# cychomatica/AudioPure

Measured on AMD Instinct MI355X. Metric: purified 1s@16kHz utterances/sec at 5 reverse steps, higher is better.
Workload: dtype f32

## Files before the change

audiopure_amd/csrc/ap_resblock_f32w.hip:

```cpp
#include "ap_common.h"

#include <type_traits>

namespace ap {

namespace {

constexpr int WC_ = 256;
constexpr int NP_ = 32;
constexpr int KCW_ = 32;
constexpr int NCH_ = WC_ / KCW_;
constexpr int XS_ = KCW_ + 4;
constexpr int XCOMP_ = NP_ * XS_;
constexpr int XBUF_ = 4 * XCOMP_;
constexpr int GS_ = WC_ + 4;
constexpr int GOFF_ = 2 * XBUF_;
constexpr int POFF_ = GOFF_ + 64 * GS_;
constexpr int PS_ = 36;
constexpr int LDS_FLOATS_ = GOFF_ + 64 * GS_;
constexpr int LDS_FLOATS_Q16_ = POFF_ + 4 * 2 * 32 * PS_;
constexpr int NCONST_ = 5 * WC_;
constexpr int DIET_CARRY_ = 2;
constexpr int DIET_CONST_ = 4;
constexpr int DIET_ROWS_ = 16;
constexpr int DIET_PK_ = 32;
constexpr int DIET_ZERO_ = 128;
constexpr int DIET_SEAM_ = 1024;
#ifndef AP_F32W_DIET
#define AP_F32W_DIET 1206
#endif
constexpr int DIET4_ = 0;
constexpr unsigned UNIT_BYTES_ = 4 * 64 * 16;
constexpr unsigned W1W_WAVE_BYTES_ = NCH_ * 4 * 4 * UNIT_BYTES_;
constexpr unsigned W2W_WAVE_BYTES_ = (WC_ / 8) * UNIT_BYTES_;

}

__global__ void pack_w1w_kernel(const float *__restrict__ w1f, float *__restrict__ out) {
  constexpr int C = WC_;
  const unsigned idx = blockIdx.x * blockDim.x + threadIdx.x;
  if (idx >= 4u * NCH_ * 4 * 4 * 4 * 64 * 4) return;
  const int e = idx & 3, lane = (idx >> 2) & 63, rt = (idx >> 8) & 3, comp = (idx >> 10) & 3, kg = (idx >> 12) & 3,
            ch = (idx >> 14) & 7, w = idx >> 17;
  const int i = lane & 31, hh = lane >> 5;
  const int c = 32 * ch + 8 * kg + 4 * hh + e;
  const int o = (rt & 1) * C + 64 * w + 32 * (rt >> 1) + i;
  const float *p = w1f + ((size_t)o * C + c) * 3;
  const double w0 = p[0], w1 = p[1], w2 = p[2];
  const double v = comp == 0 ? w0 : comp == 1 ? (w0 + w1 + w2) * 0.5 : comp == 2 ? (w0 - w1 + w2) * 0.5 : w2;
  out[idx] = (float)v;
}

__global__ void pack_w2w_kernel(const float *__restrict__ w2f, float *__restrict__ out) {
  constexpr int C = WC_;
  const unsigned idx = blockIdx.x * blockDim.x + threadIdx.x;
  if (idx >= 4u * (C / 8) * 4 * 64 * 4) return;
  const int e = idx & 3, lane = (idx >> 2) & 63, rt = (idx >> 8) & 3, kg = (idx >> 10) & 31, w = idx >> 15;
  const int i = lane & 31, hh = lane >> 5;
  const int c = 8 * kg + 4 * hh + e;
  const int o = (rt >> 1) * C + 64 * w + 32 * (rt & 1) + i;
  out[idx] = w2f[(size_t)o * C + c];
}

int launch_pack_f32w(ap_ctx *ctx, hipStream_t st) {
  const int C = ctx->C, S = ctx->S;
  const size_t n1f = (size_t)2 * C * C * 3, n2 = (size_t)(C + S) * C, n1w = (size_t)4 * 2 * C * C;
  for (int n = 0; n < ctx->NL; n++) {
    pack_w1w_kernel<<<(unsigned)((n1w + 255) / 256), 256, 0, st>>>(ctx->w1f + n * n1f, ctx->w1w + n * n1w);
    pack_w2w_kernel<<<(unsigned)((n2 + 255) / 256), 256, 0, st>>>(ctx->w2f + n * n2, ctx->w2w + n * n2);
  }
  AP_HIP(hipGetLastError());
  return 0;
}

template <bool NOH, bool SAVE = false, bool Q16 = false, int DIET = AP_F32W_DIET>
__global__ __launch_bounds__(256, 1) void resblock_f32w_kernel(
    const float *__restrict__ hin, const float *__restrict__ pt, float *__restrict__ hout, float *__restrict__ skip,
    const float *__restrict__ w1w, const float *__restrict__ b1, const float *__restrict__ w2w,
    const float *__restrict__ b2, int L, int logd, int accumulate, int ntiles, int nblk, float *__restrict__ aout) {
  constexpr int C = WC_;
  constexpr bool CARRY = (DIET & DIET_CARRY_) != 0, CONST = (DIET & DIET_CONST_) != 0;
  constexpr bool ROWS = Q16 && !NOH && (DIET & DIET_ROWS_) != 0;
  constexpr bool PK = Q16 && (DIET & DIET_PK_) != 0;
  constexpr bool ZERO = Q16 && (DIET & DIET_ZERO_) != 0;
  constexpr bool SEAM = Q16 && (DIET & DIET_SEAM_) != 0;
  static_assert(!SEAM || (CARRY && ZERO), "DIET_SEAM_ is written for the peeled first and last chunk");
  constexpr int COFF_ = Q16 ? LDS_FLOATS_Q16_ : LDS_FLOATS_;
  __shared__ __attribute__((aligned(16))) float lds[COFF_ + (CONST ? NCONST_ : 0)];

  const int tid = threadIdx.x;
  const int lane = tid & 63;
  const int wave = __builtin_amdgcn_readfirstlane(tid >> 6);
  const int j = lane & 31, hh = lane >> 5;
  const int sq = tid >> 5;
  const int d = 1 << logd;

  int t_first, t_step, t_end;
  {
    const int g = blockIdx.x, G = gridDim.x;
    if (G >= 8 && (G & 7) == 0) {
      const int xcd = g & 7, idx = g >> 3, q = nblk >> 3, r = nblk & 7;
      const int base = xcd < r ? xcd * (q + 1) : r * (q + 1) + (xcd - r) * q;
      t_first = base + idx;
      t_step = G >> 3;
      t_end = base + q + (xcd < r ? 1 : 0);
    } else {
      t_first = g;
      t_step = G;
      t_end = nblk;
    }
  }
  if (t_first >= t_end) return;
  if constexpr (CONST) {
    for (int i = tid; i < NCONST_; i += 256) lds[COFF_ + i] = i < 2 * C ? b1[i] : i < 4 * C ? b2[i - 2 * C] : pt[i - 4 * C];
    __syncthreads();
  }

  auto uni_rsrc = [&](const void *base, unsigned bytes) {
    const uint64_t hb = (uint64_t)base;
    const uint32_t lo = __builtin_amdgcn_readfirstlane((uint32_t)hb);
    const uint32_t hi = __builtin_amdgcn_readfirstlane((uint32_t)(hb >> 32));
    return __builtin_amdgcn_make_buffer_rsrc((void *)(((uint64_t)hi << 32) | lo), 0, (int)bytes, 0x00020000);
  };
  const unsigned clip_bytes = (unsigned)C * (unsigned)L * 4u;
  const __amdgpu_buffer_rsrc_t w1rs = uni_rsrc(reinterpret_cast<const char *>(w1w) + (size_t)wave * W1W_WAVE_BYTES_, W1W_WAVE_BYTES_);
  const __amdgpu_buffer_rsrc_t w2rs = uni_rsrc(reinterpret_cast<const char *>(w2w) + (size_t)wave * W2W_WAVE_BYTES_, W2W_WAVE_BYTES_);
  const unsigned lane16 = (unsigned)lane * 16u;
  const __amdgpu_buffer_rsrc_t b1rs = uni_rsrc(b1, 2u * C * 4u), b2rs = uni_rsrc(b2, 2u * C * 4u), ptrs = uni_rsrc(pt, C * 4u);
  auto ld4 = [&](const __amdgpu_buffer_rsrc_t &rs, int idx) {
    return __builtin_bit_cast(f32x4, __builtin_amdgcn_raw_buffer_load_b128(rs, (unsigned)idx * 4u, 0, 0));
  };
  int cbase = COFF_ + 64 * wave + 4 * hh;
  if constexpr (CONST && ROWS) asm volatile("" : "+v"(cbase));
  auto ld_c = [&](int idx) {
    if constexpr (ROWS) return *reinterpret_cast<const f32x4 *>(lds + cbase + (idx - 64 * wave - 4 * hh));
    else return *reinterpret_cast<const f32x4 *>(lds + COFF_ + idx);
  };
  auto ld_b1 = [&](int idx) { if constexpr (CONST) return ld_c(idx); else return ld4(b1rs, idx); };
  auto ld_b2 = [&](int idx) { if constexpr (CONST) return ld_c(2 * C + idx); else return ld4(b2rs, idx); };
  auto ld_pt = [&](int idx) { if constexpr (CONST) return ld_c(4 * C + idx); else return ld4(ptrs, idx); };

  auto load_a1 = [&](f32x4(&a)[4], unsigned unit) {
#pragma unroll
    for (int rt = 0; rt < 4; rt++)
      a[rt] = __builtin_bit_cast(f32x4, __builtin_amdgcn_raw_buffer_load_b128(w1rs, lane16 + rt * 1024u, unit * UNIT_BYTES_, 0));
  };
  auto load_a2 = [&](f32x4(&a)[4], unsigned kg) {
#pragma unroll
    for (int rt = 0; rt < 4; rt++)
      a[rt] = __builtin_bit_cast(f32x4, __builtin_amdgcn_raw_buffer_load_b128(w2rs, lane16 + rt * 1024u, kg * UNIT_BYTES_, 0));
  };

  const int col0 = d >= 32 ? j : (((j >> logd) << (logd + 1)) + (j & (d - 1)));
  const int col1 = d >= 32 ? 32 + j : col0 + d;

  int b, p0;
  __amdgpu_buffer_rsrc_t hrs;
  unsigned voff[4];
  bool tok[4];
  auto set_tile = [&](int tile) {
    b = __builtin_amdgcn_readfirstlane(tile / ntiles);
    p0 = __builtin_amdgcn_readfirstlane((tile % ntiles) * NP_);
    hrs = uni_rsrc(hin + (size_t)b * C * L, clip_bytes);
    const int p = p0 + j;
    const int tf = ((p >> logd) << (logd + 1)) + (p & (d - 1));
#pragma unroll
    for (int k = 0; k < 4; k++) {
      const int tp = tf + (k - 1) * d;
      tok[k] = (tp >= 0) && (tp < L);
      voff[k] = ((unsigned)min(max(tp, 0), L - 1) + (unsigned)(4 * sq) * (unsigned)L) * 4u;
    }
  };
    float xr[4][4];
    f32x4 ptq;
    auto issue_x = [&](int ch) {
      ptq = __builtin_bit_cast(f32x4, __builtin_amdgcn_raw_buffer_load_b128(ptrs, (unsigned)(16 * sq), ch * KCW_ * 4, 0));
#pragma unroll
      for (int cc = 0; cc < 4; cc++)
#pragma unroll
        for (int k = 0; k < 4; k++)
          xr[cc][k] = __builtin_bit_cast(float, __builtin_amdgcn_raw_buffer_load_b32(hrs, voff[k], (ch * KCW_ + cc) * L * 4, 0));
    };
    auto store_x = [&](float *dst) {
      asm volatile("" : "+v"(xr[0][0]), "+v"(xr[0][1]), "+v"(xr[0][2]), "+v"(xr[0][3]), "+v"(xr[1][0]), "+v"(xr[1][1]), "+v"(xr[1][2]),
                   "+v"(xr[1][3]), "+v"(xr[2][0]), "+v"(xr[2][1]), "+v"(xr[2][2]), "+v"(xr[2][3]), "+v"(xr[3][0]), "+v"(xr[3][1]),
                   "+v"(xr[3][2]), "+v"(xr[3][3]), "+v"(ptq));
      f32x4 c0, c1, c2, c3;
#pragma unroll
      for (int cc = 0; cc < 4; cc++) {
        const float u0 = tok[0] ? xr[cc][0] + ptq[cc] : 0.f;
        const float u1 = tok[1] ? xr[cc][1] + ptq[cc] : 0.f;
        const float u2 = tok[2] ? xr[cc][2] + ptq[cc] : 0.f;
        const float u3 = tok[3] ? xr[cc][3] + ptq[cc] : 0.f;
        c0[cc] = u0 - u2;
        c1[cc] = u1 + u2;
        c2[cc] = u2 - u1;
        c3[cc] = u3 - u1;
      }
      float *q = dst + j * XS_ + 4 * sq;
      *reinterpret_cast<f32x4 *>(q) = c0;
      *reinterpret_cast<f32x4 *>(q + XCOMP_) = c1;
      *reinterpret_cast<f32x4 *>(q + 2 * XCOMP_) = c2;
      *reinterpret_cast<f32x4 *>(q + 3 * XCOMP_) = c3;
    };

    f32x4 a[4][4];
    set_tile(t_first);
#pragma unroll
    for (int u = 0; u < 4; u++) load_a1(a[u], (unsigned)u);
    issue_x(0);

#pragma unroll 1
  for (int tile = t_first; tile < t_end; tile += t_step) {
    f32x16 acc[4][4];
    const float *xfrag = lds + j * XS_ + 4 * hh;
    f32x4 bqc[2];
    if constexpr (SEAM) {
      store_x(lds);
      __syncthreads();
      bqc[0] = *reinterpret_cast<const f32x4 *>(xfrag);
      __builtin_amdgcn_sched_barrier(0);
    }
#pragma unroll
    for (int rt = 0; rt < 4; rt++) {
      const int obase = (rt & 1) * C + 64 * wave + 32 * (rt >> 1);
#pragma unroll
      for (int q = 0; q < 4; q++) {
        const f32x4 bv = ld_b1(obase + 8 * q + 4 * hh);
        acc[1][rt][4 * q + 0] = bv[0];
        acc[1][rt][4 * q + 1] = bv[1];
        acc[1][rt][4 * q + 2] = bv[2];
        acc[1][rt][4 * q + 3] = bv[3];
      }
      if constexpr (!ZERO) {
#pragma unroll
        for (int r = 0; r < 16; r++) acc[0][rt][r] = acc[2][rt][r] = acc[3][rt][r] = 0.f;
      }
    }
    if constexpr (!SEAM) {
      store_x(lds);
      __syncthreads();
    }

    constexpr int NSTAGE = CARRY ? NCH_ - 1 : NCH_;
    auto chunk = [&](int ch, auto stage_tag, auto first_tag) __attribute__((always_inline)) {
      constexpr bool STAGE = decltype(stage_tag)::value, FIRST = decltype(first_tag)::value;
      constexpr bool XREQ = SEAM && STAGE;
      const float *xb = xfrag + (ch & 1) * XBUF_;
      if constexpr (STAGE && (!SEAM || FIRST)) issue_x(ch + 1 < NCH_ ? ch + 1 : ch);
      f32x4 bql[2];
      f32x4(&bq)[2] = SEAM ? bqc : bql;
      if constexpr (!SEAM) bq[0] = *reinterpret_cast<const f32x4 *>(xb);
      __builtin_amdgcn_sched_barrier(0);
#pragma unroll
      for (int kg = 0; kg < 4; kg++) {
#pragma unroll
        for (int comp = 0; comp < 4; comp++) {
          const int u = 4 * kg + comp;
          if (SEAM && u == 15) {
            __syncthreads();
            if constexpr (STAGE) bq[0] = *reinterpret_cast<const f32x4 *>(xfrag + ((ch + 1) & 1) * XBUF_);
            __builtin_amdgcn_sched_barrier(0);
          }
          if (XREQ && u == 13) issue_x(ch + 2 < NCH_ ? ch + 2 : NCH_ - 1);
          if (u + 1 < 16) bq[(u + 1) & 1] = *reinterpret_cast<const f32x4 *>(xb + ((u + 1) & 3) * XCOMP_ + ((u + 1) >> 2) * 8);
          if (STAGE && u == 12) store_x(lds + ((ch + 1) & 1) * XBUF_);
#pragma unroll
          for (int e = 0; e < 4; e++)
#pragma unroll
            for (int rt = 0; rt < 4; rt++) {
              if (FIRST && kg == 0 && e == 0 && comp != 1)
                acc[comp][rt] = __builtin_amdgcn_mfma_f32_32x32x2f32(a[comp][rt][e], bq[u & 1][e], f32x16{}, 0, 0, 0);
              else
                acc[comp][rt] = __builtin_amdgcn_mfma_f32_32x32x2f32(a[comp][rt][e], bq[u & 1][e], acc[comp][rt], 0, 0, 0);
            }
          if (STAGE && u == 12) {
#pragma unroll
            for (int i = 0; i < 16; i++) {
              __builtin_amdgcn_sched_group_barrier(0x008, 1, 0);
              __builtin_amdgcn_sched_group_barrier(0x002, 4, 0);
            }
            __builtin_amdgcn_sched_group_barrier(0x200, 4, 0);
          }
          if (XREQ && u == 13) {
#pragma unroll
            for (int i = 0; i < 16; i++) {
              __builtin_amdgcn_sched_group_barrier(0x008, 1, 0);
              __builtin_amdgcn_sched_group_barrier(0x020, 1, 0);
            }
          }
          __builtin_amdgcn_sched_barrier(0);
          load_a1(a[comp], (unsigned)((16 * ch + u + 4) & (16 * NCH_ - 1)));
          __builtin_amdgcn_sched_barrier(0);
        }
      }
    };
    if constexpr (ZERO) {
      chunk(0, std::true_type{}, std::true_type{});
      if constexpr (!SEAM) __syncthreads();
    }
#pragma unroll 1
    for (int ch = ZERO ? 1 : 0; ch < NSTAGE; ch++) {
      chunk(ch, std::true_type{}, std::false_type{});
      if constexpr (!SEAM) __syncthreads();
    }
#pragma unroll 1
    for (int ch = NSTAGE; ch < NCH_; ch++) {
      chunk(ch, std::false_type{}, std::false_type{});
      if constexpr (!SEAM) __syncthreads();
    }

    const int tfirst = ((p0 >> logd) << (logd + 1)) + (p0 & (d - 1));
    int tcol[2];
    tcol[0] = tfirst + j;
    tcol[1] = tfirst + (d >= 32 ? d : 32) + j;
    __amdgpu_buffer_rsrc_t ars = hrs;
    unsigned sv0 = 0, sv1 = 0;
    if constexpr (SAVE) {
      ars = uni_rsrc(aout + (size_t)b * 2 * C * L, 2u * clip_bytes);
      const int pj = p0 + j;
      const int s0 = ((pj >> logd) << (logd + 1)) + (pj & (d - 1));
      sv0 = s0 < L ? (unsigned)s0 * 4u : 0x80000000u;
      sv1 = s0 + d < L ? (unsigned)(s0 + d) * 4u : 0x80000000u;
    }
    {
      float *g0 = lds + GOFF_ + col0 * GS_ + 64 * wave + 4 * hh;
      float *g1 = lds + GOFF_ + col1 * GS_ + 64 * wave + 4 * hh;
#pragma unroll
      for (int p = 0; p < 2; p++) {
#pragma unroll
        for (int c4 = 0; c4 < 4; c4++) asm volatile("" : "+a"(acc[c4][2 * p]), "+a"(acc[c4][2 * p + 1]));
#pragma unroll
        for (int q = 0; q < 4; q++) {
          f32x4 v0, v1;
          if constexpr (PK) {
#pragma unroll
            for (int e = 0; e < 4; e += 2) {
              const int r = 4 * q + e;
              auto pr = [&](const f32x16 &t) { return f32x2{t[r], t[r + 1]}; };
              const f32x2 ta = (pr(acc[0][2 * p]) + pr(acc[1][2 * p])) + pr(acc[2][2 * p]);
              const f32x2 sa = (pr(acc[0][2 * p + 1]) + pr(acc[1][2 * p + 1])) + pr(acc[2][2 * p + 1]);
              const f32x2 tb = (pr(acc[1][2 * p]) - pr(acc[2][2 * p])) + pr(acc[3][2 * p]);
              const f32x2 sb = (pr(acc[1][2 * p + 1]) - pr(acc[2][2 * p + 1])) + pr(acc[3][2 * p + 1]);
              const f32x2 ga = gate2(ta, sa), gb = gate2(tb, sb);
              v0[e] = ga[0], v0[e + 1] = ga[1];
              v1[e] = gb[0], v1[e + 1] = gb[1];
              if constexpr (SAVE) {
                const unsigned so = ((unsigned)(64 * wave + 32 * p + 4 * hh) * (unsigned)L) * 4u;
                const u32x2 tau = __builtin_bit_cast(u32x2, ta), sau = __builtin_bit_cast(u32x2, sa);
                const u32x2 tbu = __builtin_bit_cast(u32x2, tb), sbu = __builtin_bit_cast(u32x2, sb);
#pragma unroll
                for (int i = 0; i < 2; i++) {
                  const int ro = rowoff(r + i, 0) * L * 4;
                  __builtin_amdgcn_raw_buffer_store_b32(tau[i], ars, so + sv0, ro, 0);
                  __builtin_amdgcn_raw_buffer_store_b32(sau[i], ars, so + sv0 + (unsigned)C * (unsigned)L * 4u, ro, 0);
                  __builtin_amdgcn_raw_buffer_store_b32(tbu[i], ars, so + sv1, ro, 0);
                  __builtin_amdgcn_raw_buffer_store_b32(sbu[i], ars, so + sv1 + (unsigned)C * (unsigned)L * 4u, ro, 0);
                }
              }
            }
          } else {
#pragma unroll
            for (int e = 0; e < 4; e++) {
              const int r = 4 * q + e;
              const float ta = (acc[0][2 * p][r] + acc[1][2 * p][r]) + acc[2][2 * p][r];
              const float sa = (acc[0][2 * p + 1][r] + acc[1][2 * p + 1][r]) + acc[2][2 * p + 1][r];
              const float tb = (acc[1][2 * p][r] - acc[2][2 * p][r]) + acc[3][2 * p][r];
              const float sb = (acc[1][2 * p + 1][r] - acc[2][2 * p + 1][r]) + acc[3][2 * p + 1][r];
              v0[e] = gate(ta, sa);
              v1[e] = gate(tb, sb);
              if constexpr (SAVE) {
                const unsigned so = ((unsigned)(64 * wave + 32 * p + 4 * hh) * (unsigned)L) * 4u;
                const int ro = rowoff(r, 0) * L * 4;
                __builtin_amdgcn_raw_buffer_store_b32(__builtin_bit_cast(unsigned, ta), ars, so + sv0, ro, 0);
                __builtin_amdgcn_raw_buffer_store_b32(__builtin_bit_cast(unsigned, sa), ars, so + sv0 + (unsigned)C * (unsigned)L * 4u, ro, 0);
                __builtin_amdgcn_raw_buffer_store_b32(__builtin_bit_cast(unsigned, tb), ars, so + sv1, ro, 0);
                __builtin_amdgcn_raw_buffer_store_b32(__builtin_bit_cast(unsigned, sb), ars, so + sv1 + (unsigned)C * (unsigned)L * 4u, ro, 0);
              }
            }
          }
          *reinterpret_cast<f32x4 *>(g0 + 32 * p + 8 * q) = v0;
          *reinterpret_cast<f32x4 *>(g1 + 32 * p + 8 * q) = v1;
          __builtin_amdgcn_sched_barrier(0);
        }
      }
    }

    f32x16 acc2[4][2];
    {
#pragma unroll
      for (int rt = 0; rt < 4; rt++) {
        if (NOH && rt < 2) continue;
        const int cb = 64 * wave + 32 * (rt & 1);
#pragma unroll
        for (int q = 0; q < 4; q++) {
          const int c = cb + 8 * q + 4 * hh;
          f32x4 bv = ld_b2((rt < 2 ? 0 : C) + c);
          if (rt < 2) bv += ld_pt(c);
#pragma unroll
          for (int ct = 0; ct < 2; ct++) {
            acc2[rt][ct][4 * q + 0] = bv[0];
            acc2[rt][ct][4 * q + 1] = bv[1];
            acc2[rt][ct][4 * q + 2] = bv[2];
            acc2[rt][ct][4 * q + 3] = bv[3];
          }
        }
      }
    }
    f32x4 a2[2][4];
    f32x4 a2r[4][2];
    auto load_a2r = [&](f32x4(&a)[2], unsigned soff) {
#pragma unroll
      for (int r = 0; r < 2; r++)
        a[r] = __builtin_bit_cast(f32x4, __builtin_amdgcn_raw_buffer_load_b128(w2rs, lane16 + r * 1024u, soff, 0));
    };
    if constexpr (ROWS) {
#pragma unroll
      for (int k = 0; k < 4; k++) load_a2r(a2r[k], (unsigned)k * UNIT_BYTES_);
    } else {
#pragma unroll
      for (int k = 0; k < 2; k++) load_a2(a2[k], (unsigned)k);
    }

    __builtin_amdgcn_sched_barrier(0);
    float hres[Q16 ? 1 : 2][Q16 ? 1 : 2][16];
    f32x4 hq[Q16 ? 2 : 1][Q16 ? 2 : 1][4];
    unsigned eo4[2] = {0x80000000u, 0x80000000u};
    if constexpr (Q16) {
      const int rowq = lane >> 3, cq = lane & 7;
#pragma unroll
      for (int ct = 0; ct < 2; ct++) {
        const int t = tfirst + (ct ? (d >= 32 ? d : 32) : 0) + 4 * cq;
        eo4[ct] = t < L ? ((unsigned)(64 * wave + rowq) * (unsigned)L + (unsigned)t) * 4u : 0x80000000u;
      }
      if (!NOH) {
#pragma unroll
        for (int rt = 0; rt < 2; rt++)
#pragma unroll
          for (int ct = 0; ct < 2; ct++)
#pragma unroll
            for (int p = 0; p < 4; p++)
              hq[rt][ct][p] = __builtin_bit_cast(f32x4, __builtin_amdgcn_raw_buffer_load_b128(hrs, eo4[ct], (32 * rt + 8 * p) * L * 4, 2));
      }
    }
    if (!Q16 && !NOH) {
#pragma unroll
      for (int rt = 0; rt < 2; rt++)
#pragma unroll
        for (int ct = 0; ct < 2; ct++) {
          const unsigned ev = ((unsigned)(64 * wave + 32 * rt + 4 * hh) * (unsigned)L + (unsigned)min(tcol[ct], L - 1)) * 4u;
#pragma unroll
          for (int r = 0; r < 16; r++)
            hres[rt][ct][r] = __builtin_bit_cast(float, __builtin_amdgcn_raw_buffer_load_b32(hrs, ev, rowoff(r, 0) * L * 4, 2));
        }
    }
    __syncthreads();

    typedef unsigned u32x4 __attribute__((ext_vector_type(4)));
    const float RS = 0.707106781186547524f;
    if constexpr (ROWS) {
      const __amdgpu_buffer_rsrc_t ors = uni_rsrc(hout + (size_t)b * C * L, clip_bytes);
      const __amdgpu_buffer_rsrc_t sls = uni_rsrc(skip + (size_t)b * C * L, accumulate ? clip_bytes : 0u);
      const float *gfrag = lds + GOFF_ + j * GS_ + 4 * hh;
      float *patch0 = lds + POFF_ + wave * (2 * 32 * PS_);
      const int rowq = lane >> 3, cq = lane & 7;
      f32x4 bq2[2][2];
      bq2[0][0] = *reinterpret_cast<const f32x4 *>(gfrag);
      bq2[0][1] = *reinterpret_cast<const f32x4 *>(gfrag + 32 * GS_);
      __builtin_amdgcn_sched_barrier(0);
#pragma unroll 1
      for (int kg4 = 0; kg4 < C / 8; kg4 += 4) {
#pragma unroll
        for (int k = 0; k < 4; k++) {
          const int kn = (kg4 + k + 1) & (C / 8 - 1);
          bq2[(k + 1) & 1][0] = *reinterpret_cast<const f32x4 *>(gfrag + 8 * kn);
          bq2[(k + 1) & 1][1] = *reinterpret_cast<const f32x4 *>(gfrag + 32 * GS_ + 8 * kn);
#pragma unroll
          for (int e = 0; e < 4; e++)
#pragma unroll
            for (int rt = 0; rt < 2; rt++)
#pragma unroll
              for (int ct = 0; ct < 2; ct++)
                acc2[rt][ct] = __builtin_amdgcn_mfma_f32_32x32x2f32(a2r[k][rt][e], bq2[k & 1][ct][e], acc2[rt][ct], 0, 0, 0);
          __builtin_amdgcn_sched_barrier(0);
          const int nx = kg4 + k + 4;
          load_a2r(a2r[k], nx < C / 8 ? (unsigned)nx * UNIT_BYTES_ : (unsigned)(nx - C / 8) * UNIT_BYTES_ + 2048u);
          __builtin_amdgcn_sched_barrier(0);
        }
      }
#pragma unroll
      for (int t = 0; t < 4; t++) {
        const int rt = t >> 1, ct = t & 1;
        float *patch = patch0 + (t & 1) * (32 * PS_);
        f32x4 pv[4];
#pragma unroll
        for (int k8 = 0; k8 < 8; k8++) {
          const int kg = 8 * t + k8, k = kg & 3;
          if (kg + 1 < C / 8) {
            bq2[(kg + 1) & 1][0] = *reinterpret_cast<const f32x4 *>(gfrag + 8 * (kg + 1));
            bq2[(kg + 1) & 1][1] = *reinterpret_cast<const f32x4 *>(gfrag + 32 * GS_ + 8 * (kg + 1));
          }
          if (k8 == 0) {
#pragma unroll
            for (int r = 0; r < 16; r++) patch[rowoff(r, hh) * PS_ + j] = acc2[rt][ct][r];
          }
          if (k8 == 1) {
#pragma unroll
            for (int p = 0; p < 4; p++) pv[p] = *reinterpret_cast<const f32x4 *>(patch + (rowq + 8 * p) * PS_ + 4 * cq);
          }
          if (k8 == 2) {
#pragma unroll
            for (int p = 0; p < 4; p++) {
              const f32x4 o = (hq[rt][ct][p] + pv[p]) * RS;
              __builtin_amdgcn_raw_buffer_store_b128(__builtin_bit_cast(u32x4, o), ors, eo4[ct], (32 * rt + 8 * p) * L * 4, 2);
            }
          }
#pragma unroll
          for (int e = 0; e < 4; e++)
#pragma unroll
            for (int r2 = 0; r2 < 2; r2++)
#pragma unroll
              for (int c2 = 0; c2 < 2; c2++)
                acc2[2 + r2][c2] = __builtin_amdgcn_mfma_f32_32x32x2f32(a2r[k][r2][e], bq2[kg & 1][c2][e], acc2[2 + r2][c2], 0, 0, 0);
          if (k8 == 0) {
#pragma unroll
            for (int i = 0; i < 16; i++) {
              __builtin_amdgcn_sched_group_barrier(0x008, 1, 0);
              __builtin_amdgcn_sched_group_barrier(0x002, 1, 0);
              __builtin_amdgcn_sched_group_barrier(0x200, 1, 0);
            }
          }
          if (k8 == 2) {
#pragma unroll
            for (int i = 0; i < 16; i++) {
              __builtin_amdgcn_sched_group_barrier(0x008, 1, 0);
              __builtin_amdgcn_sched_group_barrier(0x002, 2, 0);
            }
            __builtin_amdgcn_sched_group_barrier(0x040, 4, 0);
          }
          __builtin_amdgcn_sched_barrier(0);
          load_a2r(a2r[k], (unsigned)((kg + 4) & (C / 8 - 1)) * UNIT_BYTES_ + 2048u);
          if (k8 == 3) {
#pragma unroll
            for (int p = 0; p < 4; p++)
              hq[rt][ct][p] = __builtin_bit_cast(f32x4, __builtin_amdgcn_raw_buffer_load_b128(sls, eo4[ct], (32 * rt + 8 * p) * L * 4, 2));
          }
          __builtin_amdgcn_sched_barrier(0);
        }
      }
    } else {
      const float *gfrag = lds + GOFF_ + j * GS_ + 4 * hh;
#pragma unroll 1
      for (int kg4 = 0; kg4 < C / 8; kg4 += 4) {
#pragma unroll
        for (int k = 0; k < 4; k++) {
          const int kg = kg4 + k;
          f32x4 bq2[2];
          bq2[0] = *reinterpret_cast<const f32x4 *>(gfrag + 8 * kg);
          bq2[1] = *reinterpret_cast<const f32x4 *>(gfrag + 32 * GS_ + 8 * kg);
#pragma unroll
          for (int e = 0; e < 4; e++)
#pragma unroll
            for (int rt = NOH ? 2 : 0; rt < 4; rt++)
#pragma unroll
              for (int ct = 0; ct < 2; ct++)
                acc2[rt][ct] = __builtin_amdgcn_mfma_f32_32x32x2f32(a2[k & 1][rt][e], bq2[ct][e], acc2[rt][ct], 0, 0, 0);
          __builtin_amdgcn_sched_barrier(0);
          load_a2(a2[k & 1], (unsigned)((kg + 2) & (C / 8 - 1)));
          __builtin_amdgcn_sched_barrier(0);
        }
      }
    }

    const __amdgpu_buffer_rsrc_t ors = uni_rsrc((NOH ? skip : hout) + (size_t)b * C * L, clip_bytes);
    const __amdgpu_buffer_rsrc_t srs = uni_rsrc(skip + (size_t)b * C * L, clip_bytes);
    if constexpr (Q16) {
      f32x4 sk4[2][2][4];
      if constexpr (ROWS) {
      } else if (accumulate) {
#pragma unroll
        for (int rt = 0; rt < 2; rt++)
#pragma unroll
          for (int ct = 0; ct < 2; ct++)
#pragma unroll
            for (int p = 0; p < 4; p++)
              sk4[rt][ct][p] = __builtin_bit_cast(f32x4, __builtin_amdgcn_raw_buffer_load_b128(srs, eo4[ct], (32 * rt + 8 * p) * L * 4, 2));
      } else {
#pragma unroll
        for (int i = 0; i < 16; i++) (&sk4[0][0][0])[i] = f32x4{0.f, 0.f, 0.f, 0.f};
      }
      float *patch0 = lds + POFF_ + wave * (2 * 32 * PS_);
      const int rowq = lane >> 3, cq = lane & 7;
      auto leave = [&](int k, const f32x16 &tile, auto &&out4) {
        float *patch = patch0 + (k & 1) * (32 * PS_);
#pragma unroll
        for (int r = 0; r < 16; r++) patch[rowoff(r, hh) * PS_ + j] = tile[r];
#pragma unroll
        for (int p = 0; p < 4; p++) out4(p, *reinterpret_cast<const f32x4 *>(patch + (rowq + 8 * p) * PS_ + 4 * cq));
      };
      {
        if (!NOH && !ROWS) {
#pragma unroll
          for (int rt = 0; rt < 2; rt++)
#pragma unroll
            for (int ct = 0; ct < 2; ct++)
              leave(2 * rt + ct, acc2[rt][ct], [&](int p, f32x4 v) {
                const f32x4 o = (hq[rt][ct][p] + v) * RS;
                __builtin_amdgcn_raw_buffer_store_b128(__builtin_bit_cast(u32x4, o), ors, eo4[ct], (32 * rt + 8 * p) * L * 4, 2);
              });
        }
      }
      {
        set_tile(tile + t_step < t_end ? tile + t_step : tile);
        if constexpr (!CARRY) {
#pragma unroll
          for (int u = 0; u < 4; u++) load_a1(a[u], (unsigned)u);
        }
        issue_x(0);
      }
      __builtin_amdgcn_sched_barrier(0);
      {
#pragma unroll
        for (int rt = 0; rt < 2; rt++)
#pragma unroll
          for (int ct = 0; ct < 2; ct++)
            leave(2 * rt + ct, acc2[2 + rt][ct], [&](int p, f32x4 v) {
              f32x4 o;
              if constexpr (ROWS) o = hq[rt][ct][p] + v; else o = sk4[rt][ct][p] + v;
              __builtin_amdgcn_raw_buffer_store_b128(__builtin_bit_cast(u32x4, o), srs, eo4[ct], (32 * rt + 8 * p) * L * 4, 2);
            });
      }
      continue;
    }
    {
      set_tile(tile + t_step < t_end ? tile + t_step : tile);
      if constexpr (!CARRY) {
#pragma unroll
        for (int u = 0; u < 4; u++) load_a1(a[u], (unsigned)u);
      }
      issue_x(0);
    }
    __builtin_amdgcn_sched_barrier(0);

    {
      typedef unsigned u32x16 __attribute__((ext_vector_type(16)));
      const float RS = 0.707106781186547524f;
#pragma unroll
      for (int rt = NOH ? 2 : 0; rt < 4; rt++) {
#pragma unroll
        for (int ct = 0; ct < 2; ct++) {
          const int t = tcol[ct];
          const unsigned eo = t < L ? ((unsigned)(64 * wave + 32 * (rt & 1) + 4 * hh) * (unsigned)L + (unsigned)t) * 4u : 0x80000000u;
          if (rt < 2) {
#pragma unroll
            for (int r = 0; r < 16; r++)
              __builtin_amdgcn_raw_buffer_store_b32(__builtin_bit_cast(unsigned, (hres[rt & 1][ct][r] + acc2[rt][ct][r]) * RS), ors, eo,
                                                    rowoff(r, 0) * L * 4, 2);
          } else if (accumulate) {
#pragma unroll
            for (int r = 0; r < 16; r++)
              (void)__builtin_amdgcn_raw_ptr_buffer_atomic_fadd_f32(acc2[rt][ct][r], srs, (int)eo, rowoff(r, 0) * L * 4, 0);
          } else {
            const u32x16 av = __builtin_bit_cast(u32x16, acc2[rt][ct]);
#pragma unroll
            for (int r = 0; r < 16; r++)
              __builtin_amdgcn_raw_buffer_store_b32(av[r], srs, eo, rowoff(r, 0) * L * 4, 2);
          }
        }
      }
    }
  }
}

#ifdef AP_TOOLS
#define AP_F32W_AB_MASKS(X) X(0) X(2) X(4) X(6) X(22) X(54) X(150) X(182)
static int g_no_q16 = 0;
static int g_diet = AP_F32W_DIET;
#else
static constexpr int g_no_q16 = 0;
#endif

bool resblock_f32w_serves(const ap_ctx *ctx, int B, int L) {
  if (ctx->cfg.precision != AP_PREC_F32 || ctx->f32_form != 1 || ctx->C != WC_ || ctx->S != WC_ || !ctx->w1w) return false;
  if ((size_t)2 * WC_ * (size_t)L * 4 >= ((size_t)1 << 31)) return false;
  return (long long)B * ((L + 2 * NP_ - 1) / (2 * NP_) + 1) < (1ll << 31);
}

int launch_resblock_f32w(ap_ctx *ctx, int layer, const float *hin, const float *pt, float *hout, float *skip, int accumulate,
                         int B, int L, hipStream_t st, float *aout) {
  if (!resblock_f32w_serves(ctx, B, L)) return 1;
  const int g_ncu = device_cu_count();
  const int logd = layer % ctx->cfg.dilation_cycle;
  const long long d = 1ll << logd;
  const long long np = (L / (2 * d)) * d + ((L % (2 * d)) < d ? (L % (2 * d)) : d);
  const int ntiles = (int)((np + NP_ - 1) / NP_);
  const long long nblk = (long long)B * ntiles;
  if (nblk >= (1ll << 31)) return 1;
  const int C = ctx->C, S = ctx->S;
  const float *w1w = ctx->w1w + (size_t)layer * 4 * 2 * C * C;
  const float *w2w = ctx->w2w + (size_t)layer * (C + S) * C;
  const float *b1 = ctx->b1 + (size_t)layer * 2 * C;
  const float *b2 = ctx->b2 + (size_t)layer * (C + S);
  const unsigned grid = (unsigned)(nblk < g_ncu ? nblk : g_ncu);
  const bool q16 = (L & 3) == 0 && !g_no_q16;
  if (aout) {
    if (!hout) { set_error("resblock (save): needs an h' buffer"); return -22; }
    if (q16) resblock_f32w_kernel<false, true, true><<<grid, 256, 0, st>>>(hin, pt, hout, skip, w1w, b1, w2w, b2, L, logd, accumulate, ntiles, (int)nblk, aout);
    else resblock_f32w_kernel<false, true, false, DIET4_><<<grid, 256, 0, st>>>(hin, pt, hout, skip, w1w, b1, w2w, b2, L, logd, accumulate, ntiles, (int)nblk, aout);
    AP_HIP(hipGetLastError());
    return 0;
  }
#ifdef AP_TOOLS
#define AP_F32W_AB(M)                                                                                                             \
  if (hout && q16 && g_diet == M) {                                                                                               \
    resblock_f32w_kernel<false, false, true, M><<<grid, 256, 0, st>>>(hin, pt, hout, skip, w1w, b1, w2w, b2, L, logd, accumulate, \
                                                                      ntiles, (int)nblk, nullptr);                                \
    AP_HIP(hipGetLastError());                                                                                                    \
    return 0;                                                                                                                     \
  }
  AP_F32W_AB_MASKS(AP_F32W_AB)
#undef AP_F32W_AB
#endif
  if (hout && q16) resblock_f32w_kernel<false, false, true><<<grid, 256, 0, st>>>(hin, pt, hout, skip, w1w, b1, w2w, b2, L, logd, accumulate, ntiles, (int)nblk, nullptr);
  else if (hout) resblock_f32w_kernel<false, false, false, DIET4_><<<grid, 256, 0, st>>>(hin, pt, hout, skip, w1w, b1, w2w, b2, L, logd, accumulate, ntiles, (int)nblk, nullptr);
  else if (q16) resblock_f32w_kernel<true, false, true><<<grid, 256, 0, st>>>(hin, pt, hout, skip, w1w, b1, w2w, b2, L, logd, accumulate, ntiles, (int)nblk, nullptr);
  else resblock_f32w_kernel<true, false, false, DIET4_><<<grid, 256, 0, st>>>(hin, pt, hout, skip, w1w, b1, w2w, b2, L, logd, accumulate, ntiles, (int)nblk, nullptr);
  AP_HIP(hipGetLastError());
  return 0;
}

}

#ifdef AP_TOOLS
extern "C" int ap_debug_f32w_q16(int on) {
  ap::g_no_q16 = on ? 0 : 1;
  return 0;
}
extern "C" int ap_debug_resblock_f32w(ap_ctx *ctx, int layer, const float *h_in, const float *part_t_layer, float *h_out, float *skip,
                                      int accumulate, int B, int L, void *stream, float *pre_gate) {
  return ap::launch_resblock_f32w(ctx, layer, h_in, part_t_layer, h_out, skip, accumulate, B, L, (hipStream_t)stream, pre_gate);
}
extern "C" int ap_debug_f32w_diet(int mask) {
  bool known = mask == AP_F32W_DIET;
#define AP_F32W_KNOWN(M) known = known || mask == M;
  AP_F32W_AB_MASKS(AP_F32W_KNOWN)
#undef AP_F32W_KNOWN
  if (!known) return -22;
  ap::g_diet = mask;
  return 0;
}
#endif
```

Measured before the change: 59.97.

## Load dilated-conv input as 128-bit quads and interleave staging with MFMAs

Adds a DIET_QUAD_ mode, enabled by default, in which each lane fetches four consecutive time positions per tap with one 128-bit buffer load instead of sixteen scalar loads. Out-of-range taps are handled with an out-of-bounds offset rather than clamping. The mode takes part_t from the LDS copy, builds the four-component transformed inputs with packed-f32 adds, and spreads the LDS staging across the MFMA loop using sched barriers. Small dilations (1 and 2) get separate template specialisations, so the launch now dispatches on layer dilation. The goal is fewer vector memory instructions and better overlap of input staging with matrix math, at the cost of more code paths and added register pressure.

```diff
diff --git a/audiopure_amd/csrc/ap_resblock_f32w.hip b/audiopure_amd/csrc/ap_resblock_f32w.hip
--- a/audiopure_amd/csrc/ap_resblock_f32w.hip
+++ b/audiopure_amd/csrc/ap_resblock_f32w.hip
@@ -26,8 +26,9 @@
 constexpr int DIET_PK_ = 32;
 constexpr int DIET_ZERO_ = 128;
 constexpr int DIET_SEAM_ = 1024;
+constexpr int DIET_QUAD_ = 4096;
 #ifndef AP_F32W_DIET
-#define AP_F32W_DIET 1206
+#define AP_F32W_DIET 5302
 #endif
 constexpr int DIET4_ = 0;
 constexpr unsigned UNIT_BYTES_ = 4 * 64 * 16;
@@ -73,7 +74,7 @@
   return 0;
 }
 
-template <bool NOH, bool SAVE = false, bool Q16 = false, int DIET = AP_F32W_DIET>
+template <bool NOH, bool SAVE = false, bool Q16 = false, int DIET = AP_F32W_DIET, int DCLS = 4>
 __global__ __launch_bounds__(256, 1) void resblock_f32w_kernel(
     const float *__restrict__ hin, const float *__restrict__ pt, float *__restrict__ hout, float *__restrict__ skip,
     const float *__restrict__ w1w, const float *__restrict__ b1, const float *__restrict__ w2w,
@@ -84,7 +85,9 @@
   constexpr bool PK = Q16 && (DIET & DIET_PK_) != 0;
   constexpr bool ZERO = Q16 && (DIET & DIET_ZERO_) != 0;
   constexpr bool SEAM = Q16 && (DIET & DIET_SEAM_) != 0;
+  constexpr bool QUAD = Q16 && (DIET & DIET_QUAD_) != 0;
   static_assert(!SEAM || (CARRY && ZERO), "DIET_SEAM_ is written for the peeled first and last chunk");
+  static_assert(!QUAD || (SEAM && CONST), "DIET_QUAD_ takes part_t from the LDS copy and its place in the chunk from DIET_SEAM_");
   constexpr int COFF_ = Q16 ? LDS_FLOATS_Q16_ : LDS_FLOATS_;
   __shared__ __attribute__((aligned(16))) float lds[COFF_ + (CONST ? NCONST_ : 0)];
 
@@ -93,6 +96,7 @@
   const int wave = __builtin_amdgcn_readfirstlane(tid >> 6);
   const int j = lane & 31, hh = lane >> 5;
   const int sq = tid >> 5;
+  const int xc = 16 * (wave & 1) + (lane >> 2), xq = 4 * (wave >> 1) + (lane & 3);
   const int d = 1 << logd;
 
   int t_first, t_step, t_end;
@@ -139,6 +143,8 @@
   auto ld_b1 = [&](int idx) { if constexpr (CONST) return ld_c(idx); else return ld4(b1rs, idx); };
   auto ld_b2 = [&](int idx) { if constexpr (CONST) return ld_c(2 * C + idx); else return ld4(b2rs, idx); };
   auto ld_pt = [&](int idx) { if constexpr (CONST) return ld_c(4 * C + idx); else return ld4(ptrs, idx); };
+  int cptx = COFF_ + 4 * C + xc;
+  if constexpr (QUAD) asm volatile("" : "+v"(cptx));
 
   auto load_a1 = [&](f32x4(&a)[4], unsigned unit) {
 #pragma unroll
@@ -162,18 +168,30 @@
     b = __builtin_amdgcn_readfirstlane(tile / ntiles);
     p0 = __builtin_amdgcn_readfirstlane((tile % ntiles) * NP_);
     hrs = uni_rsrc(hin + (size_t)b * C * L, clip_bytes);
-    const int p = p0 + j;
+    const int p = QUAD ? p0 + 4 * xq : p0 + j;
     const int tf = ((p >> logd) << (logd + 1)) + (p & (d - 1));
 #pragma unroll
     for (int k = 0; k < 4; k++) {
-      const int tp = tf + (k - 1) * d;
+      const int tp = tf + (k - 1) * (QUAD && DCLS < 4 ? 4 : d);
       tok[k] = (tp >= 0) && (tp < L);
-      voff[k] = ((unsigned)min(max(tp, 0), L - 1) + (unsigned)(4 * sq) * (unsigned)L) * 4u;
+      if constexpr (QUAD) voff[k] = tok[k] ? ((unsigned)tp + (unsigned)xc * (unsigned)L) * 4u : 0x80000000u;
+      else voff[k] = ((unsigned)min(max(tp, 0), L - 1) + (unsigned)(4 * sq) * (unsigned)L) * 4u;
     }
   };
     float xr[4][4];
     f32x4 ptq;
+    f32x4 xv[4];
+    float ptc;
+    f32x2 su[8], sc[8];
+    float ptm[4], sc0[4], sc3[4];
     auto issue_x = [&](int ch) {
+      if constexpr (QUAD) {
+#pragma unroll
+        for (int k = 0; k < 4; k++)
+          xv[k] = __builtin_bit_cast(f32x4, __builtin_amdgcn_raw_buffer_load_b128(hrs, voff[k], ch * KCW_ * L * 4, 0));
+        ptc = lds[cptx + ch * KCW_];
+        return;
+      }
       ptq = __builtin_bit_cast(f32x4, __builtin_amdgcn_raw_buffer_load_b128(ptrs, (unsigned)(16 * sq), ch * KCW_ * 4, 0));
 #pragma unroll
       for (int cc = 0; cc < 4; cc++)
@@ -181,7 +199,62 @@
         for (int k = 0; k < 4; k++)
           xr[cc][k] = __builtin_bit_cast(float, __builtin_amdgcn_raw_buffer_load_b32(hrs, voff[k], (ch * KCW_ + cc) * L * 4, 0));
     };
+    auto stage = [&](float *dst, int g) __attribute__((always_inline)) {
+      auto pk_add = [](f32x2 x, f32x2 y) { f32x2 r; asm volatile("v_pk_add_f32 %0, %1, %2" : "=v"(r) : "v"(x), "v"(y)); return r; };
+      auto pk_sub = [](f32x2 x, f32x2 y) { f32x2 r; asm volatile("v_pk_add_f32 %0, %1, %2 neg_lo:[0,1] neg_hi:[0,1]" : "=v"(r) : "v"(x), "v"(y)); return r; };
+      auto pk_bc = [](f32x2 x, float y) {
+        f32x2 r;
+        f32x2 y2 = __builtin_nondeterministic_value(r);
+        y2[0] = y;
+        asm volatile("v_pk_add_f32 %0, %1, %2 op_sel_hi:[1,0]" : "=v"(r) : "v"(x), "v"(y2));
+        return r;
+      };
+      auto pk_sumdiff = [](f32x2 x) {
+        f32x2 r;
+        asm volatile("v_pk_add_f32 %0, %1, %1 op_sel:[0,1] op_sel_hi:[1,0] neg_hi:[0,1]" : "=v"(r) : "v"(x));
+        return r;
+      };
+      auto half = [&](int w) { return w & 1 ? f32x2{xv[w >> 1][2], xv[w >> 1][3]} : f32x2{xv[w >> 1][0], xv[w >> 1][1]}; };
+      constexpr int W0 = DCLS == 4 ? 0 : 1, NW = DCLS == 4 ? 8 : 6;
+      if (g == 0) {
+        asm volatile("" : "+v"(xv[0]), "+v"(xv[1]), "+v"(xv[2]), "+v"(xv[3]), "+v"(ptc));
+#pragma unroll
+        for (int k = 0; k < 4; k++) ptm[k] = tok[k] ? ptc : 0.f;
+      } else if (g <= 3) {
+#pragma unroll
+        for (int w = W0 + 3 * (g - 1); w < W0 + 3 * g && w < W0 + NW; w++) su[w] = pk_bc(half(w), ptm[w >> 1]);
+      } else if (g <= 7) {
+        if constexpr (DCLS == 1) {
+          const int i = g - 4;
+          sc[i] = pk_sumdiff(su[i + 2]);
+          sc0[i] = su[i + 1][1] - su[i + 2][1];
+          sc3[i] = su[i + 3][0] - su[i + 2][0];
+        } else {
+          const int h = (g - 4) >> 1;
+          auto tap = [&](int k) { return DCLS == 4 ? su[2 * k + h] : su[1 + 2 * h + k]; };
+          if (((g - 4) & 1) == 0) sc[4 * h + 0] = pk_sub(tap(0), tap(2)), sc[4 * h + 1] = pk_add(tap(1), tap(2));
+          else sc[4 * h + 2] = pk_sub(tap(2), tap(1)), sc[4 * h + 3] = pk_sub(tap(3), tap(1));
+        }
+      } else {
+        float *q = dst + 4 * xq * XS_ + xc;
+        const int w = g - 8;
+        if constexpr (DCLS == 1) {
+          const int i = w >> 1;
+          if ((w & 1) == 0) q[i * XS_] = sc0[i], q[i * XS_ + XCOMP_] = sc[i][0];
+          else q[i * XS_ + 2 * XCOMP_] = sc[i][1], q[i * XS_ + 3 * XCOMP_] = sc3[i];
+        } else {
+          const int h = w >> 2, comp = w & 3;
+          q[2 * h * XS_ + comp * XCOMP_] = sc[4 * h + comp][0];
+          q[(2 * h + 1) * XS_ + comp * XCOMP_] = sc[4 * h + comp][1];
+        }
+      }
+    };
     auto store_x = [&](float *dst) {
+      if constexpr (QUAD) {
+#pragma unroll
+        for (int g = 0; g < 16; g++) stage(dst, g);
+        return;
+      }
       asm volatile("" : "+v"(xr[0][0]), "+v"(xr[0][1]), "+v"(xr[0][2]), "+v"(xr[0][3]), "+v"(xr[1][0]), "+v"(xr[1][1]), "+v"(xr[1][2]),
                    "+v"(xr[1][3]), "+v"(xr[2][0]), "+v"(xr[2][1]), "+v"(xr[2][2]), "+v"(xr[2][3]), "+v"(xr[3][0]), "+v"(xr[3][1]),
                    "+v"(xr[3][2]), "+v"(xr[3][3]), "+v"(ptq));
@@ -264,17 +337,24 @@
           }
           if (XREQ && u == 13) issue_x(ch + 2 < NCH_ ? ch + 2 : NCH_ - 1);
           if (u + 1 < 16) bq[(u + 1) & 1] = *reinterpret_cast<const f32x4 *>(xb + ((u + 1) & 3) * XCOMP_ + ((u + 1) >> 2) * 8);
-          if (STAGE && u == 12) store_x(lds + ((ch + 1) & 1) * XBUF_);
+          if (STAGE && u == 12 && !QUAD) store_x(lds + ((ch + 1) & 1) * XBUF_);
+          auto mfma = [&](int rt, int e) __attribute__((always_inline)) {
+            if (FIRST && kg == 0 && e == 0 && comp != 1)
+              acc[comp][rt] = __builtin_amdgcn_mfma_f32_32x32x2f32(a[comp][rt][e], bq[u & 1][e], f32x16{}, 0, 0, 0);
+            else
+              acc[comp][rt] = __builtin_amdgcn_mfma_f32_32x32x2f32(a[comp][rt][e], bq[u & 1][e], acc[comp][rt], 0, 0, 0);
+          };
 #pragma unroll
           for (int e = 0; e < 4; e++)
 #pragma unroll
             for (int rt = 0; rt < 4; rt++) {
-              if (FIRST && kg == 0 && e == 0 && comp != 1)
-                acc[comp][rt] = __builtin_amdgcn_mfma_f32_32x32x2f32(a[comp][rt][e], bq[u & 1][e], f32x16{}, 0, 0, 0);
-              else
-                acc[comp][rt] = __builtin_amdgcn_mfma_f32_32x32x2f32(a[comp][rt][e], bq[u & 1][e], acc[comp][rt], 0, 0, 0);
+              mfma(rt, e);
+              if (QUAD && STAGE && u == 12) {
+                stage(lds + ((ch + 1) & 1) * XBUF_, 4 * e + rt);
+                __builtin_amdgcn_sched_barrier(0);
+              }
             }
-          if (STAGE && u == 12) {
+          if (STAGE && u == 12 && !QUAD) {
 #pragma unroll
             for (int i = 0; i < 16; i++) {
               __builtin_amdgcn_sched_group_barrier(0x008, 1, 0);
@@ -284,7 +364,7 @@
           }
           if (XREQ && u == 13) {
 #pragma unroll
-            for (int i = 0; i < 16; i++) {
+            for (int i = 0; i < (QUAD ? 4 : 16); i++) {
               __builtin_amdgcn_sched_group_barrier(0x008, 1, 0);
               __builtin_amdgcn_sched_group_barrier(0x020, 1, 0);
             }
@@ -673,12 +753,21 @@
 }
 
 #ifdef AP_TOOLS
-#define AP_F32W_AB_MASKS(X) X(0) X(2) X(4) X(6) X(22) X(54) X(150) X(182)
+#define AP_F32W_AB_MASKS(X) X(0) X(2) X(4) X(6) X(22) X(54) X(150) X(182) X(1206)
 static int g_no_q16 = 0;
 static int g_diet = AP_F32W_DIET;
 #else
 static constexpr int g_no_q16 = 0;
 #endif
+
+template <bool NOH, bool SAVE, int M, class... A>
+static void launch_q16(unsigned grid, hipStream_t st, int logd, A... args) {
+  if constexpr ((M & DIET_QUAD_) != 0) {
+    if (logd == 0) return resblock_f32w_kernel<NOH, SAVE, true, M, 1><<<grid, 256, 0, st>>>(args...);
+    if (logd == 1) return resblock_f32w_kernel<NOH, SAVE, true, M, 2><<<grid, 256, 0, st>>>(args...);
+  }
+  resblock_f32w_kernel<NOH, SAVE, true, M><<<grid, 256, 0, st>>>(args...);
+}
 
 bool resblock_f32w_serves(const ap_ctx *ctx, int B, int L) {
   if (ctx->cfg.precision != AP_PREC_F32 || ctx->f32_form != 1 || ctx->C != WC_ || ctx->S != WC_ || !ctx->w1w) return false;
@@ -705,7 +794,7 @@
   const bool q16 = (L & 3) == 0 && !g_no_q16;
   if (aout) {
     if (!hout) { set_error("resblock (save): needs an h' buffer"); return -22; }
-    if (q16) resblock_f32w_kernel<false, true, true><<<grid, 256, 0, st>>>(hin, pt, hout, skip, w1w, b1, w2w, b2, L, logd, accumulate, ntiles, (int)nblk, aout);
+    if (q16) launch_q16<false, true, AP_F32W_DIET>(grid, st, logd, hin, pt, hout, skip, w1w, b1, w2w, b2, L, logd, accumulate, ntiles, (int)nblk, aout);
     else resblock_f32w_kernel<false, true, false, DIET4_><<<grid, 256, 0, st>>>(hin, pt, hout, skip, w1w, b1, w2w, b2, L, logd, accumulate, ntiles, (int)nblk, aout);
     AP_HIP(hipGetLastError());
     return 0;
@@ -713,17 +802,17 @@
 #ifdef AP_TOOLS
 #define AP_F32W_AB(M)                                                                                                             \
   if (hout && q16 && g_diet == M) {                                                                                               \
-    resblock_f32w_kernel<false, false, true, M><<<grid, 256, 0, st>>>(hin, pt, hout, skip, w1w, b1, w2w, b2, L, logd, accumulate, \
-                                                                      ntiles, (int)nblk, nullptr);                                \
+    launch_q16<false, false, M>(grid, st, logd, hin, pt, hout, skip, w1w, b1, w2w, b2, L, logd, accumulate, ntiles, (int)nblk,    \
+                                (float *)nullptr);                                                                                \
     AP_HIP(hipGetLastError());                                                                                                    \
     return 0;                                                                                                                     \
   }
   AP_F32W_AB_MASKS(AP_F32W_AB)
 #undef AP_F32W_AB
 #endif
-  if (hout && q16) resblock_f32w_kernel<false, false, true><<<grid, 256, 0, st>>>(hin, pt, hout, skip, w1w, b1, w2w, b2, L, logd, accumulate, ntiles, (int)nblk, nullptr);
+  if (hout && q16) launch_q16<false, false, AP_F32W_DIET>(grid, st, logd, hin, pt, hout, skip, w1w, b1, w2w, b2, L, logd, accumulate, ntiles, (int)nblk, (float *)nullptr);
   else if (hout) resblock_f32w_kernel<false, false, false, DIET4_><<<grid, 256, 0, st>>>(hin, pt, hout, skip, w1w, b1, w2w, b2, L, logd, accumulate, ntiles, (int)nblk, nullptr);
-  else if (q16) resblock_f32w_kernel<true, false, true><<<grid, 256, 0, st>>>(hin, pt, hout, skip, w1w, b1, w2w, b2, L, logd, accumulate, ntiles, (int)nblk, nullptr);
+  else if (q16) launch_q16<true, false, AP_F32W_DIET>(grid, st, logd, hin, pt, hout, skip, w1w, b1, w2w, b2, L, logd, accumulate, ntiles, (int)nblk, (float *)nullptr);
   else resblock_f32w_kernel<true, false, false, DIET4_><<<grid, 256, 0, st>>>(hin, pt, hout, skip, w1w, b1, w2w, b2, L, logd, accumulate, ntiles, (int)nblk, nullptr);
   AP_HIP(hipGetLastError());
   return 0;
```

New measurement: 60.57 (median of 6 runs). 1.01x the previous value.
